# SchlomoFeng/GDN

Hardware: AMD Instinct MI355X
Metric: sliding-windows/sec forward+anomaly-score, SWaT-shape (127 sensors, W=15) (higher is better)
Workload: dtype f32; 1 GPU; BASELINE configs[2]: SWaT-shape eval forward + anomaly score; sensors=127, window=15, topk=30, dim=64, out_layer_num=1, batch=512, batches_per_launch=64, windows_per_launch=32768, storage=fp32, multi_gpu_measured=False, hip_graph=True, forward_streams=3, parallelism=single GPU

## Files before the change

gdn_amd/csrc/gdn_score.hip:

```cpp
#pragma clang fp contract(off)
#include "gdn_common.hpp"

#include <stdlib.h>

namespace {

constexpr int NQ = 6;

struct SelectArgs {
  int rank[NQ];
  double gamma[2];
  int median_pair;
  int total;
  int bracket;
};

__host__ __device__ inline void fill_select_args(SelectArgs& sa, long long t) {
  sa.median_pair = (t % 2 == 0);
  sa.rank[0] = (int)(sa.median_pair ? t / 2 - 1 : (t - 1) / 2);
  sa.rank[1] = (int)(sa.median_pair ? t / 2 : (t - 1) / 2);
  const double qs[2] = {25.0 / 100.0, 75.0 / 100.0};
  for (int h = 0; h < 2; ++h) {
    const double vi = (double)t * qs[h] + (1.0 + qs[h] * (1.0 - 1.0 - 1.0)) - 1.0;
    const double lo = floor(vi);
    long long ilo = (long long)lo, ihi = ilo + 1;
    if (ilo < 0) ilo = 0;
    if (ihi > t - 1) ihi = t - 1;
    if (ilo > t - 1) ilo = t - 1;
    sa.rank[2 + 2 * h] = (int)ilo;
    sa.rank[3 + 2 * h] = (int)ihi;
    sa.gamma[h] = vi - lo;
  }
  sa.total = (int)t;
}

struct CountArgs {
  const int* counts;
  int min_count;
  int bracket;
};

__device__ __forceinline__ const SelectArgs& select_args_for(const SelectArgs& sa, int) { return sa; }
template <typename ARGS> constexpr bool kPerSensor = false;
template <> constexpr bool kPerSensor<CountArgs> = true;

__device__ __forceinline__ const SelectArgs& select_args_for(const CountArgs& ca, int s) {
  __shared__ SelectArgs sh;
  if (threadIdx.x == 0) {
    const int c = ca.counts[s];
    if (c >= 1 && c >= ca.min_count) {
      fill_select_args(sh, c);
    } else {
      for (int q = 0; q < 6; ++q) sh.rank[q] = 0;
      sh.gamma[0] = sh.gamma[1] = 0.0;
      sh.median_pair = 0;
      sh.total = 0;
    }
    sh.bracket = ca.bracket;
  }
  __syncthreads();
  return sh;
}

constexpr unsigned long long FILLER = ~0ull;

__global__ __launch_bounds__(256) void score_keys_kernel(const float* __restrict__ pred,
                                                         const float* __restrict__ gt, int t, int n, int pitch,
                                                         double* __restrict__ keys) {
  __shared__ double tile[64][65];
  const int t0 = blockIdx.x * 64, s0 = blockIdx.y * 64;
  const int lane = threadIdx.x & 63, wv = threadIdx.x >> 6;
  for (int r = wv; r < 64; r += 4) {
    const int tick = t0 + r, s = s0 + lane;
    if (tick < t && s < n) {
      const size_t o = (size_t)tick * n + s;
      tile[r][lane] = fabs((double)pred[o] - (double)gt[o]);
    }
  }
  __syncthreads();
  for (int r = wv; r < 64; r += 4) {
    const int s = s0 + r, tick = t0 + lane;
    if (s < n && tick < pitch)
      keys[(size_t)s * pitch + tick] = tick < t ? tile[lane][r] : __longlong_as_double((long long)FILLER);
  }
}

__global__ __launch_bounds__(256) void score_keys_valid_kernel(const float* __restrict__ pred,
                                                               const float* __restrict__ gt,
                                                               const unsigned char* __restrict__ valid, int t, int n,
                                                               int pitch, double* __restrict__ keys) {
  __shared__ double tile[64][65];
  const int t0 = blockIdx.x * 64, s0 = blockIdx.y * 64;
  const int lane = threadIdx.x & 63, wv = threadIdx.x >> 6;
  for (int r = wv; r < 64; r += 4) {
    const int tick = t0 + r, s = s0 + lane;
    if (tick < t && s < n) {
      const size_t o = (size_t)tick * n + s;
      const double e = fabs((double)pred[o] - (double)gt[o]);
      tile[r][lane] = valid[o] != 0 ? e : __longlong_as_double((long long)FILLER);
    }
  }
  __syncthreads();
  for (int r = wv; r < 64; r += 4) {
    const int s = s0 + r, tick = t0 + lane;
    if (s < n && tick < pitch)
      keys[(size_t)s * pitch + tick] = tick < t ? tile[lane][r] : __longlong_as_double((long long)FILLER);
  }
}

__global__ __launch_bounds__(256) void score_key_counts_kernel(const unsigned long long* __restrict__ keys, int blocks,
                                                               int n, int pitch, int* __restrict__ counts) {
  __shared__ int total;
  const int s = blockIdx.x, tid = threadIdx.x;
  if (tid == 0) total = 0;
  __syncthreads();
  int mine = 0;
  for (int b = 0; b < blocks; ++b) {
    const unsigned long long* row = keys + ((size_t)b * n + s) * pitch;
    for (int i = tid; i < pitch; i += 256) mine += row[i] != FILLER ? 1 : 0;
  }
#pragma unroll
  for (int d = 32; d >= 1; d >>= 1) mine += __shfl_xor(mine, d);
  if ((tid & 63) == 0) atomicAdd(&total, mine);
  __syncthreads();
  if (tid == 0) counts[s] = total;
}

constexpr int SLICE = 2048;

struct SelState {
  unsigned long long prefix[NQ];
  int rem[NQ];
  int rep[NQ];
  unsigned int hist[NQ][256];
  unsigned int arrive;
  unsigned int cnt_b;
  unsigned int digits_done;
  unsigned int pad1;
};

struct KeyLayout {
  const unsigned long long* keys;
  unsigned long long* bufb;
  int blocks, n, pitch;
};

template <typename ARGS>
__global__ void select_init_kernel(SelState* __restrict__ state, const ARGS args) {
  SelState& st = state[blockIdx.x];
  const SelectArgs& sa = select_args_for(args, blockIdx.x);
  for (int i = threadIdx.x; i < NQ * 256; i += blockDim.x) (&st.hist[0][0])[i] = 0u;
  if (threadIdx.x < NQ) {
    st.prefix[threadIdx.x] = 0ull;
    st.rem[threadIdx.x] = sa.rank[threadIdx.x];
    st.rep[threadIdx.x] = 0;
  }
  if (threadIdx.x == 0) {
    st.arrive = 0u;
    st.cnt_b = 0u;
    st.digits_done = 0u;
  }
}

__device__ __forceinline__ void locate_bin(const unsigned int* h, int left0, unsigned long long pf, int shift,
                                           int lane, unsigned long long* npf, int* nrem) {
  const uint4 c4 = *reinterpret_cast<const uint4*>(h + 4 * lane);
  const int mine = (int)(c4.x + c4.y + c4.z + c4.w);
  int incl = mine;
#pragma unroll
  for (int d = 1; d < 64; d <<= 1) {
    const int up = __shfl_up(incl, d);
    if (lane >= d) incl += up;
  }
  const int excl = incl - mine;
  if (left0 >= excl && left0 < incl) {
    int left = left0 - excl, bin = 0;
    const int c[4] = {(int)c4.x, (int)c4.y, (int)c4.z, (int)c4.w};
#pragma unroll
    for (int j = 0; j < 3; ++j) {
      if (bin == j && left >= c[j]) {
        left -= c[j];
        bin = j + 1;
      }
    }
    *npf = pf | ((unsigned long long)(4 * lane + bin) << shift);
    *nrem = left;
  }
}

__device__ __forceinline__ void locate_bin512(const unsigned int* h, int left0, unsigned int code0, int lane,
                                              unsigned int* code, int* nrem) {
  const uint4 a = *reinterpret_cast<const uint4*>(h + 8 * lane);
  const uint4 b = *reinterpret_cast<const uint4*>(h + 8 * lane + 4);
  const int c[8] = {(int)a.x, (int)a.y, (int)a.z, (int)a.w, (int)b.x, (int)b.y, (int)b.z, (int)b.w};
  int mine = 0;
#pragma unroll
  for (int j = 0; j < 8; ++j) mine += c[j];
  int incl = mine;
#pragma unroll
  for (int d = 1; d < 64; d <<= 1) {
    const int up = __shfl_up(incl, d);
    if (lane >= d) incl += up;
  }
  const int excl = incl - mine;
  if (left0 >= excl && left0 < incl) {
    int left = left0 - excl, bin = 0;
#pragma unroll
    for (int j = 0; j < 7; ++j) {
      if (bin == j && left >= c[j]) {
        left -= c[j];
        bin = j + 1;
      }
    }
    *code = code0 + (unsigned int)(8 * lane + bin);
    *nrem = left;
  }
}

__device__ __forceinline__ void locate_bin2048(const unsigned int* h, int left0, int lane, unsigned int* code,
                                               int* nrem) {
  int g[8];
  int mine = 0;
#pragma unroll
  for (int j = 0; j < 8; ++j) {
    const uint4 a = *reinterpret_cast<const uint4*>(h + 32 * lane + 4 * j);
    g[j] = (int)(a.x + a.y + a.z + a.w);
    mine += g[j];
  }
  int incl = mine;
#pragma unroll
  for (int d = 1; d < 64; d <<= 1) {
    const int up = __shfl_up(incl, d);
    if (lane >= d) incl += up;
  }
  const int excl = incl - mine;
  if (left0 >= excl && left0 < incl) {
    int left = left0 - excl, grp = 0;
#pragma unroll
    for (int j = 0; j < 7; ++j) {
      if (grp == j && left >= g[j]) {
        left -= g[j];
        grp = j + 1;
      }
    }
    const uint4 a = *reinterpret_cast<const uint4*>(h + 32 * lane + 4 * grp);
    const int c[4] = {(int)a.x, (int)a.y, (int)a.z, (int)a.w};
    int bin = 0;
#pragma unroll
    for (int j = 0; j < 3; ++j) {
      if (bin == j && left >= c[j]) {
        left -= c[j];
        bin = j + 1;
      }
    }
    *code = (unsigned int)(32 * lane + 4 * grp + bin);
    *nrem = left;
  }
}

__device__ __forceinline__ void write_result(const unsigned long long* prefix, const SelectArgs& sa, int s,
                                             double* __restrict__ med_iqr) {
  double v[NQ];
  for (int q = 0; q < NQ; ++q) v[q] = __longlong_as_double((long long)prefix[q]);
  const double med = sa.median_pair ? (v[0] + v[1]) / 2.0 : v[0];
  double qv[2];
  for (int h = 0; h < 2; ++h) {
    const double a = v[2 + 2 * h], b = v[3 + 2 * h], gm = sa.gamma[h];
    const double diff = b - a;
    double r = a + diff * gm;
    if (gm >= 0.5) r = b - diff * (1.0 - gm);
    qv[h] = r;
  }
  med_iqr[2 * s] = med;
  med_iqr[2 * s + 1] = qv[1] - qv[0];
}

template <bool FROM_B, bool COMPACT>
__global__ __launch_bounds__(256) void select_pass_kernel(const KeyLayout kl, SelState* __restrict__ state,
                                                          int pass) {
  __shared__ unsigned int hist[NQ][256];
  __shared__ unsigned long long stage[COMPACT ? SLICE : 1];
  __shared__ unsigned int n_stage, out_base, ticket_s;
  __shared__ unsigned long long npf[NQ];
  __shared__ int nrem[NQ];
  const int s = blockIdx.y, g = blockIdx.x, G = gridDim.x;
  const int tid = threadIdx.x, lane = tid & 63, wv = tid >> 6;
  SelState& st = state[s];
  if (!FROM_B && !COMPACT && pass == 1 && st.digits_done >= 2u) return;
  const unsigned int slots = (unsigned int)kl.blocks * (unsigned int)kl.pitch;
  const unsigned int cnt = FROM_B ? st.cnt_b : slots;
  unsigned long long* outb = kl.bufb + (size_t)s * slots;
  const int shift = 56 - 8 * pass;
  const bool two = !FROM_B && !COMPACT && pass == 0;
  const unsigned int dref = two ? (unsigned int)(kl.keys[(size_t)s * kl.pitch] >> 56) : 0u;
  unsigned long long pf[NQ];
  bool active[NQ];
#pragma unroll
  for (int q = 0; q < NQ; ++q) {
    pf[q] = st.prefix[q];
    active[q] = st.rep[q] == q;
  }
  for (int i = tid; i < NQ * 256; i += 256) (&hist[0][0])[i] = 0u;
  if (tid == 0) n_stage = 0u;
  __syncthreads();

  for (unsigned int base = (unsigned int)g * SLICE; base < cnt; base += (unsigned int)G * SLICE) {
    const unsigned long long* in;
    unsigned int lim;
    if (FROM_B) {
      in = outb + base;
      lim = cnt - base;
    } else {
      const unsigned int blk = base / (unsigned int)kl.pitch, off = base - blk * (unsigned int)kl.pitch;
      in = kl.keys + ((size_t)blk * kl.n + s) * kl.pitch + off;
      lim = (unsigned int)kl.pitch - off;
    }
    unsigned long long key[8];
#pragma unroll
    for (int u = 0; u < 8; ++u) {
      const unsigned int i = tid + u * 256;
      key[u] = i < lim ? in[i] : FILLER;
    }
#pragma unroll
    for (int u = 0; u < 8; ++u) {
      const bool real = key[u] != FILLER;
      const unsigned int digit = (unsigned int)(key[u] >> shift) & 255u;
      const unsigned int d0 = __builtin_amdgcn_readfirstlane(digit);
      bool any = false;
#pragma unroll
      for (int q = 0; q < NQ; ++q) {
        if (!active[q]) continue;
        const bool match = real && (pass == 0 ? true : ((key[u] ^ pf[q]) >> (shift + 8)) == 0ull);
        any |= match;
        if (__all(match && digit == d0)) {
          if (lane == 0) atomicAdd(&hist[q][d0], 64u);
        } else if (match) {
          atomicAdd(&hist[q][digit], 1u);
        }
      }
      if constexpr (COMPACT) {
        if (any) stage[atomicAdd(&n_stage, 1u)] = key[u];
      }
      if (two && real && digit == dref) atomicAdd(&hist[1][(unsigned int)(key[u] >> 48) & 255u], 1u);
    }
    if constexpr (COMPACT) {
      __syncthreads();
      if (tid == 0) out_base = n_stage ? atomicAdd(&st.cnt_b, n_stage) : 0u;
      __syncthreads();
      for (unsigned int i = tid; i < n_stage; i += 256) outb[out_base + i] = stage[i];
      __syncthreads();
      if (tid == 0) n_stage = 0u;
      __syncthreads();
    }
  }
  __syncthreads();
  for (int i = tid; i < NQ * 256; i += 256) {
    const unsigned int c = (&hist[0][0])[i];
    if (c) atomicAdd(&(&st.hist[0][0])[i], c);
  }
  asm volatile("s_waitcnt vmcnt(0)" ::: "memory");
  __syncthreads();
  if (tid == 0) ticket_s = atomicAdd(&st.arrive, 1u);
  __syncthreads();
  if (ticket_s != (unsigned int)(G - 1)) return;

  for (int i = tid; i < NQ * 256; i += 256) (&hist[0][0])[i] = atomicExch(&(&st.hist[0][0])[i], 0u);
  __syncthreads();
  for (int q = wv; q < NQ; q += 4) locate_bin(hist[st.rep[q]], st.rem[q], pf[q], shift, lane, &npf[q], &nrem[q]);
  __syncthreads();
  unsigned int done = (unsigned int)pass + 1u;
  if (two) {
    bool inside = dref != 255u;
    for (int q = 0; q < NQ; ++q) inside = inside && (unsigned int)(npf[q] >> 56) == dref;
    if (inside) {
      __shared__ unsigned long long npf2[NQ];
      __shared__ int nrem2[NQ];
      for (int q = wv; q < NQ; q += 4) locate_bin(hist[1], nrem[q], npf[q], shift - 8, lane, &npf2[q], &nrem2[q]);
      __syncthreads();
      if (tid < NQ) {
        npf[tid] = npf2[tid];
        nrem[tid] = nrem2[tid];
      }
      __syncthreads();
      done = 2u;
    }
  }
  if (tid < NQ) {
    st.prefix[tid] = npf[tid];
    st.rem[tid] = nrem[tid];
    int r = tid;
    for (int q = tid - 1; q >= 0; --q)
      if (npf[q] == npf[tid]) r = q;
    st.rep[tid] = r;
  }
  if (tid == 0) {
    st.digits_done = done;
    atomicExch(&st.arrive, 0u);
  }
}

constexpr int FIN_NT = 1024;
template <bool FROM_B, typename ARGS>
__global__ __launch_bounds__(FIN_NT) void select_finish_kernel(const KeyLayout kl, SelState* __restrict__ state,
                                                            int first_pass, const ARGS args,
                                                            double* __restrict__ med_iqr) {
  __shared__ unsigned int hist[NQ][256];
  __shared__ unsigned long long prefix[NQ];
  __shared__ int rem[NQ];
  __shared__ int rep[NQ];
  const int s = blockIdx.x;
  const int tid = threadIdx.x, lane = tid & 63, wv = tid >> 6;
  const SelectArgs& sa = select_args_for(args, s);
  if constexpr (kPerSensor<ARGS>) {
    if (sa.total < 1) return;
  }
  SelState& st = state[s];
  const unsigned int slots = (unsigned int)kl.blocks * (unsigned int)kl.pitch;
  const unsigned int cnt = FROM_B ? st.cnt_b : slots;
  const unsigned long long* in = FROM_B ? kl.bufb + (size_t)s * slots : kl.keys + (size_t)s * kl.pitch;
  if (tid < NQ) {
    prefix[tid] = st.prefix[tid];
    rem[tid] = st.rem[tid];
  }
  constexpr int FK = 32;
  const bool resident = cnt <= FK * FIN_NT;
  unsigned long long key[FK];
  if (resident) {
#pragma unroll
    for (int u = 0; u < FK; ++u) {
      const unsigned int i = tid + u * FIN_NT;
      key[u] = i < cnt ? in[i] : FILLER;
    }
  }
  __syncthreads();
  for (int pass = first_pass; pass < 8; ++pass) {
    const int shift = 56 - 8 * pass;
    if (tid < NQ) {
      int r = tid;
      for (int q = tid - 1; q >= 0; --q)
        if (prefix[q] == prefix[tid]) r = q;
      rep[tid] = r;
    }
    for (int i = tid; i < NQ * 256; i += FIN_NT) (&hist[0][0])[i] = 0u;
    __syncthreads();
    unsigned long long pf[NQ];
    bool active[NQ];
#pragma unroll
    for (int q = 0; q < NQ; ++q) {
      pf[q] = prefix[q];
      active[q] = rep[q] == q;
    }
    auto tally = [&](unsigned long long k) -> bool {
      if (k == FILLER) return false;
      const unsigned int digit = (unsigned int)(k >> shift) & 255u;
      bool any = false;
#pragma unroll
      for (int q = 0; q < NQ; ++q) {
        if (!active[q]) continue;
        if (pass == 0 || ((k ^ pf[q]) >> (shift + 8)) == 0ull) {
          atomicAdd(&hist[q][digit], 1u);
          any = true;
        }
      }
      return any;
    };
    if (resident) {
#pragma unroll
      for (int u = 0; u < FK; ++u)
        if (!tally(key[u])) key[u] = FILLER;
    } else {
      for (unsigned int i = tid; i < cnt; i += FIN_NT) tally(in[i]);
    }
    __syncthreads();
    for (int q = wv; q < NQ; q += FIN_NT / 64) locate_bin(hist[rep[q]], rem[q], pf[q], shift, lane, &prefix[q], &rem[q]);
    __syncthreads();
  }
  if (tid == 0) write_result(prefix, sa, s, med_iqr);
}

constexpr int ONE_NT = 1024;
constexpr int ONE_FK = 32;
constexpr int ONE_CAP = 8192;
constexpr int ONE_CAP2 = 1024;

constexpr int BR_S = ONE_NT;
constexpr float BR_C = 2.62f;
constexpr unsigned int BR_NONE = 0xffffu;
constexpr int SPAN_BINS = 2048;
constexpr int SPAN_BELOW = SPAN_BINS;
constexpr int SPAN_CODE = SPAN_BINS + 1;

template <bool FLAT, typename ARGS>
__global__ __launch_bounds__(ONE_NT) void select_onewg_kernel(const KeyLayout kl, const ARGS args,
                                                              double* __restrict__ med_iqr, int* __restrict__ path) {
  __shared__ unsigned int hist[NQ][256];
  __shared__ unsigned int sbuf[2 * BR_S];
  __shared__ unsigned int br_below[3], br_code[NQ], br_m;
  __shared__ unsigned long long prefix[NQ];
  __shared__ unsigned long long stage[ONE_CAP];
  __shared__ unsigned long long stage2[ONE_CAP2];
  __shared__ unsigned short sidx[ONE_CAP];
  __shared__ int rem[NQ];
  __shared__ int rep[NQ];
  __shared__ unsigned int n_stage, n_stage2, dref;
  __shared__ unsigned int cnt0[2];
  const int s = blockIdx.x;
  const int tid = threadIdx.x, lane = tid & 63, wv = tid >> 6;
  const SelectArgs& sa = select_args_for(args, s);
  if constexpr (kPerSensor<ARGS>) {
    if (sa.total < 1) return;
  }
  const unsigned int slots = (unsigned int)kl.blocks * (unsigned int)kl.pitch;
#ifdef GDN_SELECT_TIMING
  const long long tick_start = wall_clock64();
#endif
  constexpr bool flat = FLAT;
  const __amdgpu_buffer_rsrc_t rsrc = __builtin_amdgcn_make_buffer_rsrc(
      const_cast<unsigned long long*>(kl.keys + (size_t)s * kl.pitch), 0, flat ? kl.pitch * 8 : 0, 0x00020000);
  auto key_full = [&](int u) -> unsigned long long {
    if constexpr (flat) {
      typedef unsigned int u32x2 __attribute__((ext_vector_type(2)));
      const u32x2 v = __builtin_amdgcn_raw_buffer_load_b64(rsrc, tid * 8, u * (ONE_NT * 8), 0);
      return ((unsigned long long)v.y << 32) | v.x;
    } else {
      const unsigned int i = tid + u * ONE_NT;
      const unsigned int blk = i / (unsigned int)kl.pitch, off = i - blk * (unsigned int)kl.pitch;
      return kl.keys[((size_t)blk * kl.n + s) * kl.pitch + off];
    }
  };
  auto key_slot = [&](unsigned int i) -> unsigned long long {
    if constexpr (flat) {
      return kl.keys[(size_t)s * kl.pitch + i];
    } else {
      const unsigned int blk = i / (unsigned int)kl.pitch, off = i - blk * (unsigned int)kl.pitch;
      return kl.keys[((size_t)blk * kl.n + s) * kl.pitch + off];
    }
  };
  const bool try_bracket = flat && sa.bracket != 0 && sa.total >= 4 * BR_S;
  unsigned int smp = 0xffffffffu;
  if constexpr (flat) {
    if (try_bracket) smp = __builtin_amdgcn_raw_buffer_load_b32(rsrc, (((unsigned int)tid * slots) / BR_S) * 8 + 4, 0, 0);
  }
  unsigned int khi[ONE_FK];
#pragma unroll
  for (int u = 0; u < ONE_FK; ++u) {
    unsigned int hi;
    if constexpr (flat) hi = __builtin_amdgcn_raw_buffer_load_b32(rsrc, tid * 8 + 4, u * (ONE_NT * 8), 0);
    else hi = tid + u * ONE_NT < slots ? (unsigned int)(key_full(u) >> 32) : 0u;
    if constexpr (flat) khi[u] = hi;
    else khi[u] = tid + u * ONE_NT < slots ? hi : 0xffffffffu;
  }
  auto stage_slots = [&](unsigned int keep) __attribute__((always_inline)) -> unsigned int {
    const int mine = __popc(keep);
    int incl = mine;
#pragma unroll
    for (int d = 1; d < 64; d <<= 1) {
      const int up = __shfl_up(incl, d);
      if (lane >= d) incl += up;
    }
    unsigned int base = 0u;
    if (lane == 63) base = atomicAdd(&n_stage, (unsigned int)incl);
    base = __shfl(base, 63);
    unsigned int pos = base + (unsigned int)(incl - mine);
    unsigned int t1 = tid;
    asm volatile("" : "+v"(t1));
#pragma unroll
    for (int u = 0; u < ONE_FK; ++u) {
      if ((keep >> u) & 1u) {
        if (pos < (unsigned int)ONE_CAP) sidx[pos] = (unsigned short)(t1 + u * ONE_NT);
        ++pos;
      }
    }
    __syncthreads();
    return n_stage;
  };
  auto finish_by_counting = [&](const unsigned long long* cand, unsigned int n, auto bucket_of, auto rank_bucket) {
    if ((unsigned int)tid < n) {
      const unsigned long long k = cand[tid];
      const auto mine = bucket_of((unsigned int)tid);
      bool wanted = false;
#pragma unroll
      for (int q = 0; q < NQ; ++q) wanted |= rank_bucket(q) == mine;
      if (wanted) {
        int less = 0, equal = 0;
        for (unsigned int j = 0; j < n; ++j) {
          const unsigned long long o = cand[j];
          if (bucket_of(j) != mine) continue;
          less += o < k ? 1 : 0;
          equal += o == k ? 1 : 0;
        }
#pragma unroll
        for (int q = 0; q < NQ; ++q) {
          const int want = rem[q];
          if (rank_bucket(q) == mine && less <= want && want < less + equal) prefix[q] = k;
        }
      }
    }
    __syncthreads();
  };
#ifdef GDN_SELECT_TIMING
  long long tick[12], btick[6] = {0, 0, 0, 0, 0, 0};
  int nt = 0;
  int br_tier = 2;
  unsigned int br_n = 0u;
#endif
  bool bracketed = false;
  if constexpr (flat) {
    if (try_bracket) {
      unsigned int* hflat = &hist[0][0];
      for (int i = tid; i < 3 * 512; i += ONE_NT) hflat[i] = 0u;
      unsigned int* shist = reinterpret_cast<unsigned int*>(stage);
      shist[tid] = 0u;
      shist[tid + ONE_NT] = 0u;
      if (tid == 0) shist[SPAN_BELOW] = 0u;
      if (tid < NQ) shist[SPAN_CODE + tid] = ~0u;
      if (tid < 3) br_below[tid] = 0u;
      if (tid < NQ) br_code[tid] = ~0u;
      if (tid == 0) {
        br_m = 0u;
        n_stage = 0u;
      }
      unsigned int v = smp;
      int pp = 0;
#pragma unroll
      for (int k = 2; k <= BR_S; k <<= 1) {
#pragma unroll
        for (int j = k >> 1; j > 0; j >>= 1) {
          unsigned int o;
          if (j >= 64) {
            sbuf[pp * BR_S + tid] = v;
            __syncthreads();
            o = sbuf[pp * BR_S + (tid ^ j)];
            pp ^= 1;
          } else {
            o = (unsigned int)__shfl_xor((int)v, j);
          }
          const bool take_min = ((tid & j) == 0) == ((tid & k) == 0);
          v = take_min ? min(v, o) : max(v, o);
        }
      }
      static_assert(BR_S == 1024, "the sorted sample ends in the first exchange buffer after ten cross-wave stages");
      sbuf[tid] = v;
      __syncthreads();
      if (v != 0xffffffffu && (tid == BR_S - 1 || sbuf[tid + 1] == 0xffffffffu)) br_m = (unsigned int)(tid + 1);
      __syncthreads();
#ifdef GDN_SELECT_TIMING
      btick[0] = wall_clock64();
#endif
    }
  }
  if constexpr (flat) {
#pragma unroll
    for (int u = 0; u < ONE_FK; ++u) khi[u] = tid + u * ONE_NT < slots ? khi[u] : 0xffffffffu;
  }
  if constexpr (flat) {
    if (try_bracket) {
      unsigned int* hflat = &hist[0][0];
      const unsigned int* sorted = sbuf;
      const int m = (int)br_m;
      if (m >= BR_S / 2) {
        const float fm = (float)m, ft = (float)sa.total;
        const int margin = (int)(BR_C * sqrtf(fm)) + 2;
        unsigned int lo[3], hi[3];
        const int first[3] = {2, 0, 4};
#pragma unroll
        for (int g = 0; g < 3; ++g) {
          const int li = (int)((float)sa.rank[first[g]] * fm / ft) - margin;
          const int ui = (int)((float)sa.rank[first[g] + 1] * fm / ft) + 1 + margin;
          lo[g] = li < 0 ? 0u : sorted[li];
          hi[g] = ui >= m ? 0x7fffffffu : sorted[ui];
        }
        unsigned int L0 = lo[0], H0 = hi[0], L1 = 0x80000000u, H1 = 0x80000000u, L2 = 0x80000000u, H2 = 0x80000000u;
        int iv_med, iv_q75;
        if (lo[1] <= H0) { H0 = hi[1]; iv_med = 0; } else { L1 = lo[1]; H1 = hi[1]; iv_med = 1; }
        if (iv_med == 0) {
          if (lo[2] <= H0) { H0 = hi[2]; iv_q75 = 0; } else { L1 = lo[2]; H1 = hi[2]; iv_q75 = 1; }
        } else {
          if (lo[2] <= H1) { H1 = hi[2]; iv_q75 = 1; } else { L2 = lo[2]; H2 = hi[2]; iv_q75 = 2; }
        }
        L0 = __builtin_amdgcn_readfirstlane(L0);
        L1 = __builtin_amdgcn_readfirstlane(L1);
        L2 = __builtin_amdgcn_readfirstlane(L2);
        const unsigned int W0 = __builtin_amdgcn_readfirstlane(H0 - L0), W1 = __builtin_amdgcn_readfirstlane(H1 - L1),
                           W2 = __builtin_amdgcn_readfirstlane(H2 - L2);
        const unsigned int S0 = W0 < 512u ? 0u : 23u - (unsigned int)__clz((int)W0),
                           S1 = W1 < 512u ? 0u : 23u - (unsigned int)__clz((int)W1),
                           S2 = W2 < 512u ? 0u : 23u - (unsigned int)__clz((int)W2);
        auto code_of = [&](unsigned int h) __attribute__((always_inline)) -> unsigned int {
          const unsigned int d0 = h - L0, d1 = h - L1, d2 = h - L2;
          unsigned int c = BR_NONE;
          if (d2 <= W2) c = 1024u + (d2 >> S2);
          if (d1 <= W1) c = 512u + (d1 >> S1);
          if (d0 <= W0) c = d0 >> S0;
          return c;
        };
        const int n_iv = iv_q75 + 1;
        unsigned int Smin = S0;
        if (n_iv > 1) Smin = min(Smin, S1);
        if (n_iv > 2) Smin = min(Smin, S2);
        const unsigned int LS = L0;
        const unsigned int WS = __builtin_amdgcn_readfirstlane(hi[2] - lo[0]);
        const unsigned int SS = WS < (unsigned int)SPAN_BINS ? 0u : 21u - (unsigned int)__clz((int)WS);
        const bool use_span = sa.bracket >= 2 && WS != 0u && SS <= Smin + 2u;
        unsigned int code[NQ];
        unsigned int n_cand = 0u;
        bool have = false, by_span = false;
        if (use_span) {
          unsigned int* shist = reinterpret_cast<unsigned int*>(stage);
          unsigned int below = 0u;
          unsigned int ssv = SS, one = 1u;
          asm volatile("" : "+v"(ssv), "+v"(one));
#pragma unroll
          for (int u = 0; u < ONE_FK; ++u) {
            const unsigned int h = khi[u];
            const unsigned int d = h - LS;
            below += h < LS ? 1u : 0u;
            if (d <= WS) atomicAdd(&shist[d >> ssv], one);
          }
#pragma unroll
          for (int d = 32; d >= 1; d >>= 1) below += __shfl_xor(below, d);
          if (lane == 0) atomicAdd(&shist[SPAN_BELOW], below);
          __syncthreads();
#ifdef GDN_SELECT_TIMING
          btick[1] = wall_clock64();
#endif
          if (wv < NQ) locate_bin2048(shist, sa.rank[wv] - (int)shist[SPAN_BELOW], lane, &shist[SPAN_CODE + wv], &rem[wv]);
          __syncthreads();
          bool inside = true;
#pragma unroll
          for (int q = 0; q < NQ; ++q) {
            code[q] = __builtin_amdgcn_readfirstlane(shist[SPAN_CODE + q]);
            inside = inside && code[q] != ~0u;
          }
          if (inside) {
            unsigned int r_lo[3], r_w[3];
            const int first[3] = {2, 0, 4};
#pragma unroll
            for (int g = 0; g < 3; ++g) {
              const unsigned int d_lo = code[first[g]] << SS, d_hi = min(((code[first[g] + 1] + 1u) << SS) - 1u, WS);
              r_lo[g] = LS + d_lo;
              r_w[g] = d_hi - d_lo;
            }
            unsigned int keep = 0u;
#pragma unroll
            for (int u = 0; u < ONE_FK; ++u) {
              const unsigned int h = khi[u];
              const bool any = (h - r_lo[0] <= r_w[0]) | (h - r_lo[1] <= r_w[1]) | (h - r_lo[2] <= r_w[2]);
              keep |= any ? (1u << u) : 0u;
            }
            asm volatile("" : "+v"(keep));
            n_cand = stage_slots(keep);
            have = by_span = n_cand <= (unsigned int)ONE_CAP2;
            if (!have) {
              __syncthreads();
              if (tid == 0) n_stage = 0u;
            }
          }
#ifdef GDN_SELECT_TIMING
          btick[2] = wall_clock64();
          br_tier = have ? 0 : 1;
#endif
        }
        if (!have) {
          unsigned int b01 = 0u, b2 = 0u;
#pragma unroll
          for (int u = 0; u < ONE_FK; ++u) {
            const unsigned int h = khi[u];
            b01 += (h < L0 ? 1u : 0u) + (h < L1 ? 0x10000u : 0u);
            b2 += h < L2 ? 1u : 0u;
            const unsigned int c = code_of(h);
            if (c != BR_NONE) atomicAdd(&hflat[c], 1u);
          }
#pragma unroll
          for (int d = 32; d >= 1; d >>= 1) {
            b01 += __shfl_xor(b01, d);
            b2 += __shfl_xor(b2, d);
          }
          if (lane == 0) {
            atomicAdd(&br_below[0], b01 & 0xffffu);
            atomicAdd(&br_below[1], b01 >> 16);
            atomicAdd(&br_below[2], b2);
          }
          __syncthreads();
#ifdef GDN_SELECT_TIMING
          btick[3] = wall_clock64();
#endif
          if (wv < NQ) {
            const int iv = wv < 2 ? iv_med : (wv < 4 ? 0 : iv_q75);
            locate_bin512(hflat + 512 * iv, sa.rank[wv] - (int)br_below[iv], 512u * (unsigned int)iv, lane,
                          &br_code[wv], &rem[wv]);
          }
          __syncthreads();
          bool inside = true;
#pragma unroll
          for (int q = 0; q < NQ; ++q) {
            code[q] = __builtin_amdgcn_readfirstlane(br_code[q]);
            inside = inside && code[q] != ~0u;
          }
          if (inside) {
            unsigned int keep = 0u;
#pragma unroll
            for (int u = 0; u < ONE_FK; ++u) {
              const unsigned int c = code_of(khi[u]);
              bool any = false;
#pragma unroll
              for (int q = 0; q < NQ; ++q) any |= c == code[q];
              keep |= any ? (1u << u) : 0u;
            }
            n_cand = stage_slots(keep);
            have = n_cand <= (unsigned int)ONE_CAP2;
          }
#ifdef GDN_SELECT_TIMING
          btick[4] = wall_clock64();
#endif
        }
#ifdef GDN_SELECT_TIMING
        br_n = n_cand;
#endif
        if (have) {
          if ((unsigned int)tid < n_cand) {
            const unsigned long long k = key_slot(sidx[tid]);
            const unsigned int hk = (unsigned int)(k >> 32);
            stage2[tid] = k;
            sidx[tid] = (unsigned short)(by_span ? (hk - LS) >> SS : code_of(hk));
          }
          __syncthreads();
          finish_by_counting(stage2, n_cand, [&](unsigned int j) { return (unsigned int)sidx[j]; },
                             [&](int q) { return code[q]; });
          bracketed = true;
        }
      }
      if (!bracketed) __syncthreads();
#ifdef GDN_SELECT_TIMING
      btick[5] = wall_clock64();
#endif
    }
  }
  if (!bracketed) {
    if (tid < NQ) {
      prefix[tid] = 0ull;
      rem[tid] = sa.rank[tid];
    }
    if (tid == 0) {
      n_stage = 0u;
      n_stage2 = 0u;
    }
    __syncthreads();
  }
#ifdef GDN_SELECT_TIMING
  tick[nt++] = wall_clock64();
#endif
  bool in_lds = false;
  bool done = bracketed;
  unsigned int n_keep = 0u;
  for (int pass = 0; pass < 8 && !done; ++pass) {
    const int shift = 56 - 8 * pass;
    if (tid < NQ) {
      int r = tid;
      for (int q = tid - 1; q >= 0; --q)
        if (prefix[q] == prefix[tid]) r = q;
      rep[tid] = r;
    }
    for (int i = tid; i < NQ * 256; i += ONE_NT) (&hist[0][0])[i] = 0u;
    if (pass == 0 && tid == 0) {
      cnt0[0] = cnt0[1] = 0u;
      dref = khi[0] >> 24;
    }
    __syncthreads();
    if (pass == 0) {
      const unsigned int dr = dref;
      unsigned int less = 0u, same = 0u;
#pragma unroll
      for (int u = 0; u < ONE_FK; ++u) {
        const unsigned int hi = khi[u];
        const unsigned int digit = hi >> 24;
        less += digit < dr ? 1u : 0u;
        same += digit == dr ? 1u : 0u;
      }
#pragma unroll
      for (int d = 32; d >= 1; d >>= 1) {
        less += __shfl_xor(less, d);
        same += __shfl_xor(same, d);
      }
      if (lane == 0) {
        atomicAdd(&cnt0[0], less);
        atomicAdd(&cnt0[1], same);
      }
      __syncthreads();
      const unsigned int tl = cnt0[0], ts = cnt0[1];
      bool inside = dr != 255u;
#pragma unroll
      for (int q = 0; q < NQ; ++q) inside = inside && (unsigned int)sa.rank[q] >= tl && (unsigned int)sa.rank[q] < tl + ts;
      if (inside) {
        if (tid < NQ) {
          prefix[tid] = (unsigned long long)dr << 56;
          rem[tid] = sa.rank[tid] - (int)tl;
        }
        __syncthreads();
#ifdef GDN_SELECT_TIMING
        tick[nt++] = wall_clock64();
#endif
        continue;
      }
    }
    if (!in_lds && pass < 3) {
      const unsigned int sh = 24u - 8u * (unsigned int)pass;
#pragma nounroll
      for (int q = 0; q < NQ; ++q) {
        if (rep[q] != q) continue;
        const unsigned int pfh = (unsigned int)(prefix[q] >> 32);
        unsigned int* hq = hist[q];
#pragma unroll
        for (int u = 0; u < ONE_FK; ++u) {
          const unsigned int hi = khi[u];
          const bool real = (int)hi >= 0;
          const unsigned int digit = (hi >> sh) & 255u;
          if (pass == 0) {
            const unsigned int d0 = __builtin_amdgcn_readfirstlane(digit);
            if (__all(real && digit == d0)) {
              if (lane == 0) atomicAdd(&hq[d0], 64u);
            } else if (real) {
              atomicAdd(&hq[digit], 1u);
            }
          } else if (real && ((hi ^ pfh) >> (sh + 8u)) == 0u) {
            atomicAdd(&hq[digit], 1u);
          }
        }
      }
    } else if (!in_lds) {
#pragma nounroll
      for (int q = 0; q < NQ; ++q) {
        if (rep[q] != q) continue;
        const unsigned long long pfq = prefix[q];
        unsigned int* hq = hist[q];
#pragma unroll 4
        for (int u = 0; u < ONE_FK; ++u) {
          const bool real = (int)khi[u] >= 0;
          const unsigned long long k = real ? key_full(u) : FILLER;
          const unsigned int digit = (unsigned int)(k >> shift) & 255u;
          if (real && ((k ^ pfq) >> (shift + 8)) == 0ull) atomicAdd(&hq[digit], 1u);
        }
      }
    } else {
#pragma nounroll
      for (int q = 0; q < NQ; ++q) {
        if (rep[q] != q) continue;
        const unsigned long long pfq = prefix[q];
        unsigned int* hq = hist[q];
        for (unsigned int i = tid; i < n_keep; i += ONE_NT) {
          const unsigned long long k = stage[i];
          const unsigned int digit = (unsigned int)(k >> shift) & 255u;
          if (((k ^ pfq) >> (shift + 8)) == 0ull) atomicAdd(&hq[digit], 1u);
        }
      }
    }
    __syncthreads();
    for (int q = wv; q < NQ; q += ONE_NT / 64)
      locate_bin(hist[rep[q]], rem[q], prefix[q], shift, lane, &prefix[q], &rem[q]);
    __syncthreads();
    if (pass == 1) {
      unsigned int p16[NQ];
#pragma unroll
      for (int q = 0; q < NQ; ++q) {
        p16[q] = __builtin_amdgcn_readfirstlane((unsigned int)(prefix[q] >> 48));
#pragma unroll
        for (int r = 0; r < q; ++r)
          if (p16[r] == p16[q]) p16[q] = 0x10000u;
      }
      unsigned int keep = 0u;
#pragma unroll
      for (int u = 0; u < ONE_FK; ++u) {
        const unsigned int h16 = khi[u] >> 16;
        bool any = false;
#pragma unroll
        for (int q = 0; q < NQ; ++q) any |= h16 == p16[q];
        keep |= any ? (1u << u) : 0u;
      }
      n_keep = stage_slots(keep);
      in_lds = n_keep <= (unsigned int)ONE_CAP;
      if (in_lds) {
        for (unsigned int i = tid; i < n_keep; i += ONE_NT) stage[i] = key_slot(sidx[i]);
        __syncthreads();
      }
    }
    if (pass == 2 && in_lds) {
      for (unsigned int i = tid; i < n_keep; i += ONE_NT) {
        const unsigned long long k = stage[i];
        bool any = false;
#pragma unroll
        for (int q = 0; q < NQ; ++q) any |= ((k ^ prefix[q]) >> 40) == 0ull;
        if (any) {
          const unsigned int at = atomicAdd(&n_stage2, 1u);
          if (at < (unsigned int)ONE_CAP2) stage2[at] = k;
        }
      }
      __syncthreads();
      const unsigned int n2 = n_stage2;
      if (n2 <= (unsigned int)ONE_CAP2) {
        finish_by_counting(stage2, n2, [&](unsigned int j) { return stage2[j] >> 40; },
                           [&](int q) { return prefix[q] >> 40; });
        done = true;
      }
    }
#ifdef GDN_SELECT_TIMING
    tick[nt++] = wall_clock64();
#endif
  }
#ifdef GDN_SELECT_TIMING
  if (tid == 0 && s == 1 && bracketed && br_tier == 0)
    printf("onewg bracket ticks(10ns): sample sort (under the row load) %lld count+histogram %lld locate+stage %lld "
           "re-read+finish %lld candidates %u tier one-span\n",
           btick[0] - tick_start, btick[1] - btick[0], btick[2] - btick[1], btick[5] - btick[2], br_n);
  else if (tid == 0 && s == 1 && bracketed)
    printf("onewg bracket ticks(10ns): sample sort (under the row load) %lld count+histogram %lld locate+stage %lld "
           "re-read+finish %lld candidates %u tier three-interval (one-span before it: %lld)\n",
           btick[0] - tick_start, btick[3] - (br_tier == 1 ? btick[2] : btick[0]), btick[4] - btick[3],
           btick[5] - btick[4], br_n, br_tier == 1 ? btick[2] - btick[0] : 0ll);
  else if (tid == 0 && s == 1)
    printf("onewg ticks(10ns): load %lld p0 %lld p1+compact %lld p2+finish %lld (passes run %d) survivors %u / %u\n",
           tick[0] - tick_start, tick[1] - tick[0], tick[2] - tick[1], tick[3] - tick[2], nt - 1, n_keep, n_stage2);
#endif
  if (tid == 0) {
    write_result(prefix, sa, s, med_iqr);
    if (path) path[s] = bracketed ? 0 : 1;
  }
}

constexpr int RUN = 8;

template <bool GAPS>
__global__ __launch_bounds__(256) void score_smooth_max_kernel(
    const float* __restrict__ pred, const float* __restrict__ gt, const double* __restrict__ med_iqr,
    int t, int n, int first_tick, const float* __restrict__ halo_pred, const float* __restrict__ halo_gt,
    double* __restrict__ scores, double* __restrict__ anomaly, const unsigned char* __restrict__ valid,
    const unsigned char* __restrict__ halo_valid) {
  __shared__ double best[4][RUN];
  const int lane = threadIdx.x & 63, wv = threadIdx.x >> 6;
  const int wpb = blockDim.x >> 6;
  const int nruns = (t + RUN - 1) / RUN;
  for (int run = blockIdx.x * wpb + wv; run < nruns; run += gridDim.x * wpb) {
    const int t0 = run * RUN, t1 = min(t, t0 + RUN);
    for (int s0 = 0; s0 < n; s0 += 128) {
      const int sa_ = s0 + lane, sb_ = s0 + 64 + lane;
      const bool la = sa_ < n, lb = sb_ < n;
      const int ca = la ? sa_ : n - 1, cb = lb ? sb_ : n - 1;
      const double meda = med_iqr[2 * ca], dena = 1.0 / (fabs(med_iqr[2 * ca + 1]) + 1e-2);
      const double medb = med_iqr[2 * cb], denb = 1.0 / (fabs(med_iqr[2 * cb + 1]) + 1e-2);
      const int g0 = first_tick + t0;
      float pa[RUN + 3], ga[RUN + 3], pb[RUN + 3], gb[RUN + 3];
      unsigned oka = 0u, okb = 0u;
#pragma unroll
      for (int u = 0; u < RUN + 3; ++u) {
        const int tt = t0 - 3 + u;
        const bool halo = tt < 0;
// ... 384 lines not shown
```

Baseline: 152.9 million windows/s.

## Restructure in-block selection with DPP swaps, ballot compaction and packed prefix scan

The 2048-bin locate now loads a strided layout and packs two 16-bit group sums per register, so four prefix scans run in parallel instead of eight sequential group reductions. Bitonic sample-sort exchanges inside a wave use DPP and permlane swaps in place of generic shuffles, and the sample count comes from a ballot plus atomic add, which removes one block barrier. Span candidate staging switches from a mask plus block-wide scan to per-iteration wave ballots with atomic slot reservation. A barrier is added after the sample load. The 16-bit packing assumes group counts below 65536, and the atomic staging changes the order of candidates.

```diff
diff --git a/gdn_amd/csrc/gdn_score.hip b/gdn_amd/csrc/gdn_score.hip
--- a/gdn_amd/csrc/gdn_score.hip
+++ b/gdn_amd/csrc/gdn_score.hip
@@ -219,31 +219,37 @@
 
 __device__ __forceinline__ void locate_bin2048(const unsigned int* h, int left0, int lane, unsigned int* code,
                                                int* nrem) {
-  int g[8];
-  int mine = 0;
+  unsigned int p[4], incl[4];
+#pragma unroll
+  for (int a = 0; a < 4; ++a) {
+    const uint4 x = *reinterpret_cast<const uint4*>(h + 4 * (lane + 64 * (2 * a)));
+    const uint4 y = *reinterpret_cast<const uint4*>(h + 4 * (lane + 64 * (2 * a + 1)));
+    p[a] = (x.x + x.y + x.z + x.w) | ((y.x + y.y + y.z + y.w) << 16);
+    incl[a] = p[a];
+  }
+#pragma unroll
+  for (int d = 1; d < 64; d <<= 1) {
+#pragma unroll
+    for (int a = 0; a < 4; ++a) {
+      const unsigned int up = (unsigned int)__shfl_up((int)incl[a], d);
+      if (lane >= d) incl[a] += up;
+    }
+  }
+  int start = 0, hit = -1, left = 0;
 #pragma unroll
   for (int j = 0; j < 8; ++j) {
-    const uint4 a = *reinterpret_cast<const uint4*>(h + 32 * lane + 4 * j);
-    g[j] = (int)(a.x + a.y + a.z + a.w);
-    mine += g[j];
-  }
-  int incl = mine;
-#pragma unroll
-  for (int d = 1; d < 64; d <<= 1) {
-    const int up = __shfl_up(incl, d);
-    if (lane >= d) incl += up;
-  }
-  const int excl = incl - mine;
-  if (left0 >= excl && left0 < incl) {
-    int left = left0 - excl, grp = 0;
-#pragma unroll
-    for (int j = 0; j < 7; ++j) {
-      if (grp == j && left >= g[j]) {
-        left -= g[j];
-        grp = j + 1;
-      }
-    }
-    const uint4 a = *reinterpret_cast<const uint4*>(h + 32 * lane + 4 * grp);
+    const int sh = 16 * (j & 1);
+    const int mine = (int)((p[j >> 1] >> sh) & 0xffffu);
+    const int excl = start + (int)((incl[j >> 1] >> sh) & 0xffffu) - mine;
+    if (left0 >= excl && left0 < excl + mine) {
+      hit = j;
+      left = left0 - excl;
+    }
+    start += (int)((__builtin_amdgcn_readlane((int)incl[j >> 1], 63) >> sh) & 0xffff);
+  }
+  if (hit >= 0) {
+    const int grp = lane + 64 * hit;
+    const uint4 a = *reinterpret_cast<const uint4*>(h + 4 * grp);
     const int c[4] = {(int)a.x, (int)a.y, (int)a.z, (int)a.w};
     int bin = 0;
 #pragma unroll
@@ -253,7 +259,7 @@
         bin = j + 1;
       }
     }
-    *code = (unsigned int)(32 * lane + 4 * grp + bin);
+    *code = (unsigned int)(4 * grp + bin);
     *nrem = left;
   }
 }
@@ -490,6 +496,28 @@
 constexpr int SPAN_BELOW = SPAN_BINS;
 constexpr int SPAN_CODE = SPAN_BINS + 1;
 
+__device__ __forceinline__ unsigned int lane_xor(unsigned int v, int j, int lane) {
+  typedef unsigned int u32x2 __attribute__((ext_vector_type(2)));
+  const int iv = (int)v;
+  switch (j) {
+    case 1: return (unsigned int)__builtin_amdgcn_update_dpp(iv, iv, 0xB1, 0xf, 0xf, false);
+    case 2: return (unsigned int)__builtin_amdgcn_update_dpp(iv, iv, 0x4E, 0xf, 0xf, false);
+    case 4: {
+      const int m = __builtin_amdgcn_update_dpp(iv, iv, 0x141, 0xf, 0xf, false);
+      return (unsigned int)__builtin_amdgcn_update_dpp(m, m, 0x1B, 0xf, 0xf, false);
+    }
+    case 8: return (unsigned int)__builtin_amdgcn_update_dpp(iv, iv, 0x128, 0xf, 0xf, false);
+    case 16: {
+      const u32x2 r = __builtin_amdgcn_permlane16_swap(v, v, false, false);
+      return (lane & 16) ? r.x : r.y;
+    }
+    default: {
+      const u32x2 r = __builtin_amdgcn_permlane32_swap(v, v, false, false);
+      return (lane & 32) ? r.x : r.y;
+    }
+  }
+}
+
 template <bool FLAT, typename ARGS>
 __global__ __launch_bounds__(ONE_NT) void select_onewg_kernel(const KeyLayout kl, const ARGS args,
                                                               double* __restrict__ med_iqr, int* __restrict__ path) {
@@ -539,7 +567,10 @@
   const bool try_bracket = flat && sa.bracket != 0 && sa.total >= 4 * BR_S;
   unsigned int smp = 0xffffffffu;
   if constexpr (flat) {
-    if (try_bracket) smp = __builtin_amdgcn_raw_buffer_load_b32(rsrc, (((unsigned int)tid * slots) / BR_S) * 8 + 4, 0, 0);
+    if (try_bracket) {
+      smp = __builtin_amdgcn_raw_buffer_load_b32(rsrc, (((unsigned int)tid * slots) / BR_S) * 8 + 4, 0, 0);
+      __builtin_amdgcn_s_barrier();
+    }
   }
   unsigned int khi[ONE_FK];
 #pragma unroll
@@ -633,16 +664,16 @@
             o = sbuf[pp * BR_S + (tid ^ j)];
             pp ^= 1;
           } else {
-            o = (unsigned int)__shfl_xor((int)v, j);
+            o = lane_xor(v, j, lane);
           }
           const bool take_min = ((tid & j) == 0) == ((tid & k) == 0);
           v = take_min ? min(v, o) : max(v, o);
         }
       }
       static_assert(BR_S == 1024, "the sorted sample ends in the first exchange buffer after ten cross-wave stages");
+      const unsigned long long real = __ballot(v != 0xffffffffu);
+      if (lane == 0) atomicAdd(&br_m, (unsigned int)__popcll(real));
       sbuf[tid] = v;
-      __syncthreads();
-      if (v != 0xffffffffu && (tid == BR_S - 1 || sbuf[tid + 1] == 0xffffffffu)) br_m = (unsigned int)(tid + 1);
       __syncthreads();
 #ifdef GDN_SELECT_TIMING
       btick[0] = wall_clock64();
@@ -741,15 +772,27 @@
               r_lo[g] = LS + d_lo;
               r_w[g] = d_hi - d_lo;
             }
-            unsigned int keep = 0u;
+            unsigned int t1 = tid;
+            asm volatile("" : "+v"(t1));
 #pragma unroll
             for (int u = 0; u < ONE_FK; ++u) {
               const unsigned int h = khi[u];
               const bool any = (h - r_lo[0] <= r_w[0]) | (h - r_lo[1] <= r_w[1]) | (h - r_lo[2] <= r_w[2]);
-              keep |= any ? (1u << u) : 0u;
+              const unsigned long long mask = __ballot(any);
+              if (mask != 0ull) {
+                const int first = __ffsll((long long)mask) - 1;
+                unsigned int base = 0u;
+                if (lane == first) base = atomicAdd(&n_stage, (unsigned int)__popcll(mask));
+                base = (unsigned int)__builtin_amdgcn_readlane((int)base, first);
+                if (any) {
+                  const unsigned int pos = base + __builtin_amdgcn_mbcnt_hi((unsigned int)(mask >> 32),
+                                                                            __builtin_amdgcn_mbcnt_lo((unsigned int)mask, 0u));
+                  if (pos < (unsigned int)ONE_CAP) sidx[pos] = (unsigned short)(t1 + u * ONE_NT);
+                }
+              }
             }
-            asm volatile("" : "+v"(keep));
-            n_cand = stage_slots(keep);
+            __syncthreads();
+            n_cand = n_stage;
             have = by_span = n_cand <= (unsigned int)ONE_CAP2;
             if (!have) {
               __syncthreads();
```

Result: no change. 153.7 million windows/s, median of 6 (+0.5%).
